# dylkot/cNMF

Hardware: AMD Instinct MI355X
Metric: NMF restarts/sec (50000x2000xK5..13) (higher is better)
Workload: dtype f32 (exact integer f16 plane x 2 f16 planes with per-row exponent, f32 accumulate)

## Files before the change

### cnmf_amd/csrc/gemm_host.hip.h

```cpp
#pragma once

struct GemmPlan { int variant; int mw; int jw; };

template <int MTW, int WM, int WN, bool NN, int TBK = BK>
static hipError_t launch_gemm_t(hipStream_t st, const float* A, int lda, const float* B, int ldb,
                                float* C, int ldc, long long cstride, int KC, int Ktot, int J,
                                int nsplit)
{
    constexpr int MW = WM * MTW * 32, JW = WN * 32;
    const int Kper = round_up((Ktot + nsplit - 1) / nsplit, BK);
    dim3 grid((J + JW - 1) / JW, KC / MW, nsplit);
    constexpr size_t lds = gemm_lds_bytes<MTW, WM, WN, NN, TBK>();
    {
        if (hipError_t e_ = dyn_lds_optin((const void*)gemm_kernel<MTW, WM, WN, NN, TBK>, (int)lds)) return e_;
    }
    gemm_kernel<MTW, WM, WN, NN, TBK><<<grid, 256, lds, st>>>(A, lda, B, ldb, C, ldc, cstride, Kper,
                                                             Ktot, J);
    return hipGetLastError();
}

static const CdKnobs k_default_knobs;
static thread_local const CdKnobs* g_knobs = &k_default_knobs;
struct KnobScope {
    const CdKnobs* prev;
    explicit KnobScope(const cnmf_ctx* ctx) : prev(g_knobs) { g_knobs = &ctx->knobs; }
    ~KnobScope() { g_knobs = prev; }
    KnobScope(const KnobScope&) = delete;
    KnobScope& operator=(const KnobScope&) = delete;
};

template <bool NN>
static hipError_t launch_gemm(hipStream_t st, int variant, const float* A, int lda, const float* B,
                              int ldb, float* C, int ldc, long long cstride, int KC, int Ktot,
                              int J, int nsplit)
{
#define GO(MTW, WM, WN) \
    return launch_gemm_t<MTW, WM, WN, NN>(st, A, lda, B, ldb, C, ldc, cstride, KC, Ktot, J, nsplit)
    if (variant == 0) variant = 2;
    if (variant == 1 && KC < 128) variant = (KC >= 64) ? 3 : 2;
    if (variant == 3 && KC < 64) variant = 2;
    switch (variant) {
        case 1:
            if (KC % 256 == 0 && KC >= 256 && g_knobs->s_mtw2) GO(2, 4, 1);
            GO(1, 4, 1);
        case 3:
            if (KC % 128 == 0) GO(2, 2, 2);
            GO(1, 2, 2);
        default:
            if (KC % 128 == 0) GO(4, 1, 4);
            if (KC % 64 == 0) GO(2, 1, 4);
            GO(1, 1, 4);
    }
#undef GO
}

static SplitInfo psum_info(int nsplit, long long stride, const double* colscale)
{
    SplitInfo sp{nullptr, reinterpret_cast<const unsigned char*>(colscale), (int)(stride >> 20), (int)(stride & ((1 << 20) - 1)), nsplit};
    return sp;
}

static hipError_t launch_sweep(hipStream_t st, int nslots, float* V, int ldv, int L, const float* P,
                               const float* gram, const SlotDesc* slots, float l1, float* gram_part,
                               double* viol_part, int chunks, int parts, int want_gram, int kmax, int tiers,
                               SplitInfo sp = SplitInfo{nullptr, nullptr, 1, 1, 1},
                               float* rmax_part = nullptr, const double* rmax_scale = nullptr, bool psum = false,
                               PlaneOut po = PlaneOut{nullptr, nullptr, 0, 0})
{
    dim3 grid(parts, nslots);
    if (po.dst) {
        if (psum || (rmax_part && rmax_scale) || (tiers & 8)) return hipErrorInvalidValue;
        const size_t pl = sweep_lds_bytes(kmax, true);
        const int kgp = sweep_kg(kmax);
        if (hipError_t e_ = dyn_lds_optin((const void*)sweep_kernel<0, false, false, true>, (int)sweep_lds_bytes(KSMALL, true))) return e_;
        if (hipError_t e_ = dyn_lds_optin((const void*)sweep_kernel<1, false, false, true>, (int)sweep_lds_bytes(KSMALL, true))) return e_;
        if (hipError_t e_ = dyn_lds_optin((const void*)sweep_kernel<2, false, false, true>, (int)sweep_lds_bytes(KSMALL, true))) return e_;
#define CNMF_SWEEP_PLN(T_) sweep_kernel<T_, false, false, true><<<grid, 256, pl, st>>>(V, ldv, L, P, sp, gram, slots, l1, gram_part, viol_part, chunks, want_gram, kgp, kmax, rmax_part, nullptr, po)
        if (tiers & 1) CNMF_SWEEP_PLN(0);
        if (tiers & 2) CNMF_SWEEP_PLN(1);
        if (tiers & 4) CNMF_SWEEP_PLN(2);
#undef CNMF_SWEEP_PLN
        return hipGetLastError();
    }
    {
        if (hipError_t e_ = dyn_lds_optin((const void*)sweep_kernel<0, false>, (int)sweep_lds_bytes(KSMALL))) return e_;
        if (hipError_t e_ = dyn_lds_optin((const void*)sweep_kernel<1, false>, (int)sweep_lds_bytes(KSMALL))) return e_;
        if (hipError_t e_ = dyn_lds_optin((const void*)sweep_kernel<2, false>, (int)sweep_lds_bytes(KSMALL))) return e_;
        if (hipError_t e_ = dyn_lds_optin((const void*)sweep_kernel<0, true>, (int)sweep_lds_bytes(KSMALL))) return e_;
        if (hipError_t e_ = dyn_lds_optin((const void*)sweep_kernel<1, true>, (int)sweep_lds_bytes(KSMALL))) return e_;
        if (hipError_t e_ = dyn_lds_optin((const void*)sweep_kernel<2, true>, (int)sweep_lds_bytes(KSMALL))) return e_;
    }
    const size_t lds = sweep_lds_bytes(kmax);
    const int kg = sweep_kg(kmax);
#define CNMF_SWEEP(T_, R_) sweep_kernel<T_, R_><<<grid, 256, lds, st>>>(V, ldv, L, P, sp, gram, slots, l1, gram_part, viol_part, chunks, want_gram, kg, kmax, rmax_part, rmax_scale)
#define CNMF_SWEEP_PSUM(T_) sweep_kernel<T_, true, true><<<grid, 256, lds, st>>>(V, ldv, L, P, sp, gram, slots, l1, gram_part, viol_part, chunks, want_gram, kg, kmax, rmax_part, rmax_scale)
    if (psum) {
        {
            if (hipError_t e_ = dyn_lds_optin((const void*)sweep_kernel<0, true, true>, (int)sweep_lds_bytes(KSMALL))) return e_;
            if (hipError_t e_ = dyn_lds_optin((const void*)sweep_kernel<1, true, true>, (int)sweep_lds_bytes(KSMALL))) return e_;
            if (hipError_t e_ = dyn_lds_optin((const void*)sweep_kernel<2, true, true>, (int)sweep_lds_bytes(KSMALL))) return e_;
        }
        if (tiers & 1) CNMF_SWEEP_PSUM(0);
        if (tiers & 2) CNMF_SWEEP_PSUM(1);
        if (tiers & 4) CNMF_SWEEP_PSUM(2);
    } else if (rmax_part && rmax_scale) {
        if (tiers & 1) CNMF_SWEEP(0, true);
        if (tiers & 2) CNMF_SWEEP(1, true);
        if (tiers & 4) CNMF_SWEEP(2, true);
    } else {
        if (tiers & 1) CNMF_SWEEP(0, false);
        if (tiers & 2) CNMF_SWEEP(1, false);
        if (tiers & 4) CNMF_SWEEP(2, false);
    }
#undef CNMF_SWEEP_PSUM
#undef CNMF_SWEEP
    if (tiers & 8) {
        if (psum) return hipErrorInvalidValue;
        const size_t blds = sweep_big_lds_bytes();
        const int bchunks = chunks;
        const dim3 gbig(parts, nslots);
        if (rmax_part && rmax_scale) {
            if (hipError_t e_ = dyn_lds_optin((const void*)sweep_big_kernel<true>, (int)blds)) return e_;
            sweep_big_kernel<true><<<gbig, 256, blds, st>>>(V, ldv, L, P, sp, gram, slots, l1, viol_part, bchunks, rmax_part, rmax_scale);
        } else {
            if (hipError_t e_ = dyn_lds_optin((const void*)sweep_big_kernel<false>, (int)blds)) return e_;
            sweep_big_kernel<false><<<gbig, 256, blds, st>>>(V, ldv, L, P, sp, gram, slots, l1, viol_part, bchunks, nullptr, nullptr);
        }
        if (want_gram)
            gram_big_kernel<<<gbig, 256, 0, st>>>(V, ldv, L, slots, gram_part, bchunks, kmax, (rmax_part && !rmax_scale) ? rmax_part : nullptr);
    }
    return hipGetLastError();
}

struct StreamK {
    bool on = false;
    int MG = 1, T = 0, nk = 0, P = 0, mw = 128;
    std::vector<unsigned char> split;
};

static StreamK plan_streamk(int KC, int N_pad, int G_pad, int n_wg_slots)
{
    StreamK sk;
    if (KC % 128 != 0 || g_knobs->no_streamk) return sk;
    sk.MG = KC / sk.mw;
    sk.T = sk.MG * (N_pad / 128);
    sk.nk = G_pad / BK;
    sk.P = n_wg_slots;
    if (sk.T <= sk.P) sk.P = n_wg_slots / 2;
    if (sk.T <= sk.P || sk.T % sk.P == 0) return sk;
    sk.on = true;
    sk.split.assign(sk.T, 0);
    const long long U = (long long)sk.T * sk.nk;
    for (int p = 1; p < sk.P; ++p) {
        const long long b = U * p / sk.P;
        if (b % sk.nk) sk.split[b / sk.nk] = 1;
    }
    return sk;
}

static hipError_t launch_streamk_passA(hipStream_t st, const StreamK& sk, const float* A, int lda,
                                       const float* B, int ldb, float* C0, float* C1, int ldc, int Jtot)
{
    constexpr size_t lds = gemm_lds_bytes<4, 1, 4, false>();
    {
        if (hipError_t e_ = dyn_lds_optin((const void*)gemm_streamk_kernel<4, 1, 4, false>, (int)lds)) return e_;
    }
    gemm_streamk_kernel<4, 1, 4, false><<<sk.P, 256, lds, st>>>(A, lda, B, ldb, C0, C1, ldc, sk.MG, sk.T,
                                                               sk.nk, Jtot);
    return hipGetLastError();
}

static hipError_t launch_reduce_splits(hipStream_t st, float* P, int nsplit, long long split_stride,
                                       long long n_floats, const double* colscale = nullptr, int ld = 1)
{
    if (nsplit <= 1 && !colscale) return hipSuccess;
    const long long nv = n_floats / 4;
    reduce_splits_kernel<<<(unsigned)((nv + 255) / 256), 256, 0, st>>>(P, nsplit, split_stride, P, nv, colscale, ld);
    return hipGetLastError();
}


static hipError_t launch_split3(hipStream_t st, const float* src, int ld, int rows, int K, unsigned char* dst, int TR,
                                const double* kscale = nullptr)
{
    if (rows % 64 == 0 && K % 64 == 0 && TR % 64 == 0) {
        dim3 grid(K / 64, rows / 64);
        split3_tiled_kernel<<<grid, 256, 0, st>>>(src, ld, K, TR, (unsigned short*)dst, kscale);
        return hipGetLastError();
    }
    const long long total = (long long)rows * (K / 16);
    split3_kernel<<<(unsigned)((total + 255) / 256), 256, 0, st>>>(src, ld, rows, K, TR, (unsigned short*)dst, kscale);
    return hipGetLastError();
}

static int gemm3_mode() { return g_knobs->gemm3; }
static int gemm3_wg_slots(const CdKnobs& k)
{
    if (k.wg_slots >= 32 && k.gemm3 >= 2) return k.wg_slots;
    return k.gemm3 >= 2 ? 256 : 512;
}
static int gemm3_jw() { return G3_JW; }

static hipError_t launch_gemm3(hipStream_t st, const unsigned char* A3, const unsigned char* B3, int Kb,
                               float* C, int ldc, long long cstride, int KC, int Jpad, int nsplit)
{
    {
        if (hipError_t e_ = dyn_lds_optin((const void*)gemm3_kernel, G3_LDS_BYTES)) return e_;
        if (hipError_t e_ = dyn_lds_optin((const void*)gemm3g_kernel, G3G_LDS_BYTES)) return e_;
    }
    const int kb_per = (Kb + nsplit - 1) / nsplit;
    dim3 grid(Jpad / gemm3_jw(), KC / G3_MW, (Kb + kb_per - 1) / kb_per);
    if (gemm3_mode() >= 2)
        gemm3g_kernel<<<grid, 512, G3G_LDS_BYTES, st>>>(A3, B3, Kb, C, ldc, cstride, kb_per);
    else
        gemm3_kernel<<<grid, 256, G3_LDS_BYTES, st>>>(A3, B3, Kb, C, ldc, cstride, kb_per);
    return hipGetLastError();
}


static hipError_t launch_split3_finalize(hipStream_t st, const float* src, int ld, int rows, int K, unsigned char* dst,
                                         int TR, const double* kscale, const FinalizeArgs& fa, int nslots, int fin_y)
{
    const int bx = K / 64, by = rows / 64;
    split3_finalize_kernel<<<bx * by + nslots * fin_y, 256, 0, st>>>(src, ld, K, TR, (unsigned short*)dst, kscale, bx, by,
                                                                  fa, fin_y);
    return hipGetLastError();
}

static hipError_t launch_split2h_finalize(hipStream_t st, const float* src, int ld, int rows, int K, unsigned char* dst,
                                          int TR, const double* kscale, const float* rmax_part, int parts,
                                          float* inv_scale, const FinalizeArgs& fa, int nslots, int fin_y,
                                          SplitFused fu = SplitFused{nullptr, nullptr});

struct StreamK3 {
    bool on = false;
    int T = 0, Kb = 0, P = 0, MG = 1;
    std::vector<unsigned char> flags;
};

static StreamK3 plan_streamk3(int KC, int N_pad, int G_pad, int n_wg_slots, int jw, int unit = 1)
{
    StreamK3 sk;
    sk.MG = KC / G3_MW;
    sk.T = sk.MG * (N_pad / jw);
    sk.Kb = G_pad / (G3_BK * unit);
    sk.P = n_wg_slots;
    if (sk.T < sk.P / 2 + sk.P / 4 || sk.P > 2 * sk.T || g_knobs->no_streamk) return sk;
    sk.on = true;
    sk.flags.assign(sk.T, 0);
    const long long U = (long long)sk.T * sk.Kb;
    const int NJ = sk.T / sk.MG;
    for (int p = 1; p < sk.P; ++p) {
        const long long b = U * p / sk.P;
        if (b % sk.Kb) {
            const int o = (int)(b / sk.Kb);
            unsigned char& f = sk.flags[(o % NJ) * sk.MG + o / NJ];
            f = f ? 3 : 1;
        }
    }
    return sk;
}
// ... 352 lines not shown
```

### cnmf_amd/csrc/kernels_sweep.hip.h

```cpp
#pragma once
#include <hip/hip_runtime.h>
#include "kernels_gemm.hip.h"
#include "kernels_gemm2h.hip.h"

namespace cnmf {

constexpr int KMAX = 128;
constexpr int KSMALL = 64;
constexpr int GRAM_LD = KMAX;
constexpr int GRAM_SZ = KMAX * KMAX;

static inline int sweep_kg(int kmax) { return kmax <= 16 ? 16 : (kmax <= 32 ? 32 : 64); }
static inline int sweep_wstride(int kmax) { return sweep_kg(kmax) + 1; }
static inline size_t sweep_lds_bytes(int kmax, bool planes = false)
{
    const int kg = sweep_kg(kmax);
    if (planes)
        return sweep_lds_bytes(kmax, false) + sizeof(float) * (size_t)(4 * kg * 64 + kg);
    return sizeof(float) * (size_t)(kg * (kg + 4) + 8 + 256 + 4 * (kg == 16 ? 32 : 64) * sweep_wstride(kmax));
}

struct SlotDesc {
    int off;
    int k;
    int active;
    int iter;
    int restart;
    int pad_;
    double viol;
    double viol_init;
    double viol_last;
};

typedef float f32x4 __attribute__((ext_vector_type(4)));

struct SplitInfo {
    const float* plane1;
    const unsigned char* split;
    int tile_rows, tile_cols, mgroups;
    const float* plane2 = nullptr;
};

struct PlaneOut {
    unsigned short* dst;
    const int* shift;
    int Kb, TR;
};

#ifndef CNMF_SWEEP_PF
#define CNMF_SWEEP_PF 0
#endif
template <int KP, bool RMX, bool PSUM = false, bool PLN = false>
__device__ __forceinline__ void sweep_body(
    float* __restrict__ V, int ldv, int L, const float* __restrict__ P, const SplitInfo& sp,
    const float* __restrict__ gram, const SlotDesc& sd, int slot, float l1_reg,
    float* __restrict__ gram_part, double* __restrict__ viol_part,
    int chunks_per_block, int want_gram, float* lds, int kg, int gld,
    float* __restrict__ rmax_part, const double* __restrict__ rmax_scale, const PlaneOut& po = PlaneOut{nullptr, nullptr, 0, 0})
{
    constexpr int GMODE = (KP <= 16) ? 0 : ((KP <= 32) ? 1 : 2);
    constexpr int GR = (GMODE == 0) ? 16 : ((GMODE == 1) ? 32 : 64);
    const int gs = kg + 4, wstride = kg + 1;
    float* Gsb = lds;
    double* vred = reinterpret_cast<double*>(lds + kg * gs);
    float* rmx = lds + kg * gs + 8;
    float* Wsb = rmx + 256;
    unsigned* Tpl = reinterpret_cast<unsigned*>(Wsb + 4 * (kg == 16 ? 32 : 64) * (kg + 1));
    int* shl = reinterpret_cast<int*>(Tpl + 4 * kg * 64);
#define GS(t_, r_) Gsb[(t_) * gs + (r_)]
    constexpr int SR = (GMODE == 0) ? 32 : 64;
#define WS(wv_, r_, c_) Wsb[((wv_) * SR + (r_)) * wstride + (c_)]
    const int k = sd.k, off = sd.off;
    const int tid = threadIdx.x, lane = tid & 63, wave = tid >> 6;
    for (int e = tid; e < KP * KP; e += 256) {
        const int r = e / KP, c = e % KP;
        GS(r, c) = (r < k && c < k) ? gram[(size_t)slot * GRAM_SZ + r * GRAM_LD + c] : 0.f;
    }
    if constexpr (PLN) { if (tid < KP) shl[tid] = po.shift[off + min(tid, k - 1)]; }
    __syncthreads();

    f32x16 gacc[GMODE == 2 ? 4 : 1];
    f32x4 gacc4 = {0.f, 0.f, 0.f, 0.f};
#pragma unroll
    for (int a = 0; a < (GMODE == 2 ? 4 : 1); ++a)
#pragma unroll
        for (int r = 0; r < 16; ++r) gacc[a][r] = 0.f;
    float viol = 0.f;
    float mx[RMX ? KP : 1];
#pragma unroll
    for (int c = 0; c < (RMX ? KP : 1); ++c) mx[c] = 0.f;

    constexpr bool PF = (CNMF_SWEEP_PF != 0) && !PSUM;
    float wn[PF ? KP : 1], pn[PF ? KP : 1];
    if constexpr (PF) {
        const int rowc0 = min((int)(blockIdx.x * chunks_per_block) * 256 + tid, L - 1);
#pragma unroll
        for (int c = 0; c < KP; ++c) {
            const size_t idx = (size_t)(off + min(c, k - 1)) * ldv + rowc0;
            wn[c] = V[idx];
            pn[c] = P[idx];
        }
    }
    for (int ch = 0; ch < chunks_per_block; ++ch) {
        const int row = (blockIdx.x * chunks_per_block + ch) * 256 + tid;
        const bool live = row < L;
        int cut0 = 0, cut1 = 0;
        int mg_edge = 1 << 30;
        if (!PSUM && sp.plane1) {
            const int rt = __builtin_amdgcn_readfirstlane(min(row, L - 1) / sp.tile_rows);
            const int g0 = off / sp.tile_cols, g1 = (off + k - 1) / sp.tile_cols;
            mg_edge = (g0 + 1) * sp.tile_cols;
            cut0 = sp.split[rt * sp.mgroups + g0];
            cut1 = sp.split[rt * sp.mgroups + g1];
        }
        float w[KP], p[KP];
        float dsc = 1.0f;
        if constexpr (RMX) { if (rmax_scale) dsc = (float)rmax_scale[min(row, L - 1)]; }
        {
            const int rowc = min(row, L - 1);
            if constexpr (PF) {
#pragma unroll
                for (int c = 0; c < KP; ++c) { w[c] = wn[c]; p[c] = pn[c]; }
                if (ch + 1 < chunks_per_block) {
                    const int rown = min(row + 256, L - 1);
#pragma unroll
                    for (int c = 0; c < KP; ++c) {
                        const size_t idx = (size_t)(off + min(c, k - 1)) * ldv + rown;
                        wn[c] = V[idx];
                        pn[c] = P[idx];
                    }
                }
            } else {
#pragma unroll
            for (int c = 0; c < KP; ++c) {
                const size_t idx = (size_t)(off + min(c, k - 1)) * ldv + rowc;
                w[c] = V[idx];
                p[c] = P[idx];
            }
            }
            if constexpr (PSUM) {
                const int nsplit = sp.mgroups;
                const size_t stride = (size_t)sp.tile_rows * (1u << 20) + (size_t)sp.tile_cols;
                constexpr int U = KP <= 16 ? 8 : (KP <= 32 ? 2 : 1);
                for (int s = 1; s < nsplit; s += U) {
                    float q[U][KP];
#pragma unroll
                    for (int u = 0; u < U; ++u) {
                        const int ss = min(s + u, nsplit - 1);
#pragma unroll
                        for (int c = 0; c < KP; ++c)
                            q[u][c] = P[ss * stride + (size_t)(off + min(c, k - 1)) * ldv + rowc];
                    }
#pragma unroll
                    for (int u = 0; u < U; ++u)
                        if (s + u < nsplit) {
#pragma unroll
                            for (int c = 0; c < KP; ++c) p[c] += q[u][c];
                        }
                }
                const double* colscale = reinterpret_cast<const double*>(sp.split);
                if (colscale) {
                    const double cs = colscale[rowc];
#pragma unroll
                    for (int c = 0; c < KP; ++c) p[c] = (float)((double)p[c] * cs);
                }
            }
            if ((cut0 | cut1) & 1) {
                float qq[KP];
#pragma unroll
                for (int c = 0; c < KP; ++c) {
                    const size_t idx = (size_t)(off + min(c, k - 1)) * ldv + rowc;
                    qq[c] = sp.plane1[idx];
                }
#pragma unroll
                for (int c = 0; c < KP; ++c) {
                    const int cut = ((off + c) < mg_edge) ? cut0 : cut1;
                    p[c] += (cut & 1) ? qq[c] : 0.f;
                }
            }
            if ((cut0 | cut1) & 2) {
                float qq[KP];
#pragma unroll
                for (int c = 0; c < KP; ++c) {
                    const size_t idx = (size_t)(off + min(c, k - 1)) * ldv + rowc;
                    qq[c] = sp.plane2[idx];
                }
#pragma unroll
                for (int c = 0; c < KP; ++c) {
                    const int cut = ((off + c) < mg_edge) ? cut0 : cut1;
                    p[c] += (cut & 2) ? qq[c] : 0.f;
                }
            }
#pragma unroll
            for (int c = 0; c < KP; ++c) {
                const bool on = live && (c < k);
                w[c] = on ? w[c] : 0.f;
                p[c] = on ? (p[c] - l1_reg) : 0.f;
            }
        }
        if (live) {
#pragma unroll
            for (int t = 0; t < KP; ++t) {
                if (t < k) {
                    float grad = -p[t];
#pragma unroll
                    for (int r = 0; r < KP; ++r) grad = fmaf(GS(t, r), w[r], grad);
                    const float pg = (w[t] == 0.f) ? fminf(0.f, grad) : grad;
                    viol += fabsf(pg);
                    const float hess = GS(t, t);
                    if (hess != 0.f) w[t] = fmaxf(w[t] - grad / hess, 0.f);
                }
            }
#pragma unroll
            for (int c = 0; c < KP; ++c)
                if (c < k) V[(size_t)(off + c) * ldv + row] = w[c];
            if constexpr (RMX) {
#pragma unroll
                for (int c = 0; c < KP; ++c) mx[c] = fmaxf(mx[c], w[c] * dsc);
            }
        }
        if (want_gram) {
            if constexpr (GMODE == 0) {
                const int li = lane & 15, q = lane >> 4;
#pragma unroll
                for (int hf = 0; hf < 2; ++hf) {
                    if ((lane >> 5) == hf) {
#pragma unroll
                        for (int c = 0; c < GR; ++c) WS(wave, lane & 31, c) = (c < KP) ? w[c < KP ? c : 0] : 0.f;
                    }
                    __builtin_amdgcn_wave_barrier();
#pragma unroll
                    for (int s = 0; s < 8; ++s) {
                        const float a = WS(wave, 4 * s + q, li);
                        gacc4 = __builtin_amdgcn_mfma_f32_16x16x4f32(a, a, gacc4, 0, 0, 0);
                    }
                    __builtin_amdgcn_wave_barrier();
                }
            } else if constexpr (GMODE == 1) {
#pragma unroll
                for (int c = 0; c < GR; ++c) WS(wave, lane, c) = (c < KP) ? w[c < KP ? c : 0] : 0.f;
                __builtin_amdgcn_wave_barrier();
                const int li = lane & 31, h = lane >> 5;
#pragma unroll 8
                for (int s = 0; s < 32; ++s) {
                    const float a = WS(wave, 2 * s + h, li);
                    gacc[0] = __builtin_amdgcn_mfma_f32_32x32x2f32(a, a, gacc[0], 0, 0, 0);
                }
            } else {
#pragma unroll
                for (int c = 0; c < GR; ++c) WS(wave, lane, c) = (c < KP) ? w[c < KP ? c : 0] : 0.f;
                __builtin_amdgcn_wave_barrier();
                const int li = lane & 31, h = lane >> 5;
#pragma unroll 4
                for (int s = 0; s < 32; ++s) {
                    const float a0 = WS(wave, 2 * s + h, li), a1 = WS(wave, 2 * s + h, 32 + li);
                    gacc[0] = __builtin_amdgcn_mfma_f32_32x32x2f32(a0, a0, gacc[0], 0, 0, 0);
                    gacc[1] = __builtin_amdgcn_mfma_f32_32x32x2f32(a0, a1, gacc[1], 0, 0, 0);
                    gacc[2] = __builtin_amdgcn_mfma_f32_32x32x2f32(a1, a0, gacc[2], 0, 0, 0);
                    gacc[3] = __builtin_amdgcn_mfma_f32_32x32x2f32(a1, a1, gacc[3], 0, 0, 0);
                }
            }
            __builtin_amdgcn_wave_barrier();
        }
        if constexpr (PLN) {
            unsigned* tw = Tpl + wave * (kg * 64);
#pragma unroll
            for (int c = 0; c < KP; ++c) {
                if (c < k) {
                    const float y = ldexpf(w[c], shl[c]);
                    unsigned short hb, mb;
                    split2h(y, hb, mb);
                    tw[c * 64 + lane] = (unsigned)hb | ((unsigned)mb << 16);
                }
            }
            __builtin_amdgcn_wave_barrier();
            const int kb0 = ((blockIdx.x * chunks_per_block + ch) * 256 + wave * 64) >> 4;
            for (int item = lane; item < 8 * k; item += 64) {
                const int c = item >> 3, b = (item >> 1) & 3, hf = item & 1;
                if (kb0 + b >= po.Kb) continue;
                const u32x4 d0 = *reinterpret_cast<const u32x4*>(tw + c * 64 + b * 16 + hf * 8);
                const u32x4 d1 = *reinterpret_cast<const u32x4*>(tw + c * 64 + b * 16 + hf * 8 + 4);
                u32x4 oh, om;
                oh.x = (d0.x & 0xffffu) | (d0.y << 16); oh.y = (d0.z & 0xffffu) | (d0.w << 16);
                oh.z = (d1.x & 0xffffu) | (d1.y << 16); oh.w = (d1.z & 0xffffu) | (d1.w << 16);
                om.x = (d0.x >> 16) | (d0.y & 0xffff0000u); om.y = (d0.z >> 16) | (d0.w & 0xffff0000u);
                om.z = (d1.x >> 16) | (d1.y & 0xffff0000u); om.w = (d1.z >> 16) | (d1.w & 0xffff0000u);
                const int r = off + c, tr = r / po.TR, rin = r % po.TR, swz = (rin >> 2) & 3;
                unsigned short* g = po.dst + (((size_t)tr * po.Kb + (kb0 + b)) * po.TR + rin) * 32;
                *reinterpret_cast<u32x4*>(g + ((0 + hf) ^ swz) * 8) = oh;
                *reinterpret_cast<u32x4*>(g + ((2 + hf) ^ swz) * 8) = om;
            }
            __builtin_amdgcn_wave_barrier();
        }
    }

    if constexpr (RMX) {
#pragma unroll
        for (int c = 0; c < KP; ++c) {
            float v = mx[c];
#pragma unroll
            for (int o = 32; o > 0; o >>= 1) v = fmaxf(v, __shfl_xor(v, o, 64));
            if (lane == 0) rmx[wave * 64 + c] = v;
        }
    }
    double dv = (double)viol;
#pragma unroll
    for (int o = 32; o > 0; o >>= 1) dv += __shfl_xor(dv, o, 64);
    if (lane == 0) vred[wave] = dv;

    __syncthreads();
    float* gred = Wsb;
    if (want_gram) {
        if constexpr (GMODE == 0) {
            const int li = lane & 15, q = lane >> 4;
#pragma unroll
            for (int r = 0; r < 4; ++r) gred[(wave * GR + 4 * q + r) * (GR + 1) + li] = gacc4[r];
        } else {
            const int li = lane & 31, h = lane >> 5;
#pragma unroll
            for (int a = 0; a < (GMODE == 2 ? 4 : 1); ++a)
#pragma unroll
                for (int r = 0; r < 16; ++r) {
                    const int rr = (a >> 1) * 32 + (r & 3) + 8 * (r >> 2) + 4 * h;
                    gred[(wave * GR + rr) * (GR + 1) + (a & 1) * 32 + li] = gacc[a][r];
                }
        }
    }
    __syncthreads();
    if (want_gram) {
        float* gp = gram_part + ((size_t)slot * gridDim.x + blockIdx.x) * (size_t)(gld * gld);
        for (int e = tid; e < k * k; e += 256) {
            const int r = e / k, c = e % k;
            gp[r * gld + c] = gred[(0 * GR + r) * (GR + 1) + c] + gred[(1 * GR + r) * (GR + 1) + c] +
                              gred[(2 * GR + r) * (GR + 1) + c] + gred[(3 * GR + r) * (GR + 1) + c];
        }
    }
    if (tid == 0)
        viol_part[(size_t)slot * gridDim.x + blockIdx.x] = vred[0] + vred[1] + vred[2] + vred[3];
    if (rmax_part && tid < k && (RMX || want_gram)) {
        float v;
        if constexpr (RMX) v = fmaxf(fmaxf(rmx[tid], rmx[64 + tid]), fmaxf(rmx[128 + tid], rmx[192 + tid]));
        else v = sqrtf(gred[(0 * GR + tid) * (GR + 1) + tid] + gred[(1 * GR + tid) * (GR + 1) + tid] +
                       gred[(2 * GR + tid) * (GR + 1) + tid] + gred[(3 * GR + tid) * (GR + 1) + tid]) * 1.0001f;
        rmax_part[(size_t)(off + tid) * gridDim.x + blockIdx.x] = v;
    }
#undef WS
#undef GS
}

template <int TIER, bool RMX = false, bool PSUM = false, bool PLN = false>
__global__ __launch_bounds__(256) __attribute__((amdgpu_waves_per_eu((TIER == 0 && !RMX && !PLN) ? 5 : (TIER == 0 && !RMX ? 4 : 1), 8))) void sweep_kernel(
    float* __restrict__ V, int ldv, int L,
    const float* __restrict__ P,
    SplitInfo sp,
    const float* __restrict__ gram,
    const SlotDesc* __restrict__ slots,
    float l1_reg,
    float* __restrict__ gram_part,
    double* __restrict__ viol_part,
    int chunks_per_block, int want_gram, int kg, int gld,
    float* __restrict__ rmax_part = nullptr,
    const double* __restrict__ rmax_scale = nullptr,
    PlaneOut po = PlaneOut{nullptr, nullptr, 0, 0})
{
    const int slot = blockIdx.y;
    const SlotDesc sd = slots[slot];
    if (!sd.active) return;
    extern __shared__ __attribute__((aligned(16))) float sweep_lds[];
#define CNMF_SW(KP_)                                                                              \
        sweep_body<KP_, RMX, PSUM, PLN>(V, ldv, L, P, sp, gram, sd, slot, l1_reg, gram_part, viol_part, \
                        chunks_per_block, want_gram, sweep_lds, kg, gld, rmax_part, rmax_scale, po);
    const int k = sd.k;
    if (TIER == 0) {
        if (k > 16) return;
        switch ((k + 3) / 4) {
            case 1: CNMF_SW(4) break;   case 2: CNMF_SW(8) break;   case 3: CNMF_SW(12) break;
            case 4: CNMF_SW(16) break;  default: break;
        }
    } else if (TIER == 1) {
        if (k <= 16 || k > 32) return;
        switch ((k + 3) / 4) {
            case 5: CNMF_SW(20) break;  case 6: CNMF_SW(24) break;
            case 7: CNMF_SW(28) break;  case 8: CNMF_SW(32) break;  default: break;
        }
    } else {
        if (k <= 32) return;
        if (k <= 48) { CNMF_SW(48) } else if (k <= 64) { CNMF_SW(64) }
    }
#undef CNMF_SW
}

constexpr int KBIG = 128;
constexpr int KBIG_GS = KBIG + 4;
static inline size_t sweep_big_lds_bytes() { return sizeof(float) * (size_t)(KBIG * KBIG_GS + 2 * 256 * 33 + 4 * KBIG + 16); }

template <bool RMX>
__global__ __launch_bounds__(256) void sweep_big_kernel(
    float* __restrict__ V, int ldv, int L, const float* __restrict__ P, SplitInfo sp, const float* __restrict__ gram,
    const SlotDesc* __restrict__ slots, float l1_reg, double* __restrict__ viol_part, int chunks_per_block,
    float* __restrict__ rmax_part, const double* __restrict__ rmax_scale)
{
    const int slot = blockIdx.y;
    const SlotDesc sd = slots[slot];
    if (!sd.active || sd.k <= KSMALL) return;
    extern __shared__ __attribute__((aligned(16))) float sweep_lds[];
    float* Gs = sweep_lds;
    float* Pl = Gs + KBIG * KBIG_GS;
    float* Wl = Pl + 256 * 33;
    float* rmx = Wl + 256 * 33;
    double* vred = reinterpret_cast<double*>(rmx + 4 * KBIG);
    const int k = sd.k, off = sd.off;
    const int tid = threadIdx.x, lane = tid & 63, wave = tid >> 6;
    for (int e = tid; e < KBIG * KBIG; e += 256) {
        const int r = e / KBIG, c = e % KBIG;
        Gs[r * KBIG_GS + c] = (r < k && c < k) ? gram[(size_t)slot * GRAM_SZ + r * GRAM_LD + c] : 0.f;
    }
    if (RMX) for (int e = tid; e < 4 * KBIG; e += 256) rmx[e] = 0.f;
    __syncthreads();
    float viol = 0.f;
    float* pl = Pl + tid * 33;
    float* wl = Wl + tid * 33;
    for (int ch = 0; ch < chunks_per_block; ++ch) {
        const int row = (blockIdx.x * chunks_per_block + ch) * 256 + tid;
        const bool live = row < L;
        const int rowc = min(row, L - 1);
        int cut0 = 0, cut1 = 0, mg_edge = 1 << 30;
        if (sp.plane1) {
            const int rt = __builtin_amdgcn_readfirstlane(rowc / sp.tile_rows);
            const int g0 = off / sp.tile_cols, g1 = (off + k - 1) / sp.tile_cols;
            mg_edge = (g0 + 1) * sp.tile_cols;
            cut0 = sp.split[rt * sp.mgroups + g0];
            cut1 = sp.split[rt * sp.mgroups + g1];
        }
        float w[KBIG];
#pragma unroll
        for (int c = 0; c < KBIG; ++c) {
            const float v = V[(size_t)(off + min(c, k - 1)) * ldv + rowc];
            w[c] = (live && c < k) ? v : 0.f;
        }
        float dsc = 1.0f;
        if (RMX && rmax_scale) dsc = (float)rmax_scale[rowc];
#pragma unroll
        for (int tb = 0; tb < KBIG / 32; ++tb) {
            if (tb * 32 < k) {
#pragma unroll
                for (int rr = 0; rr < 32; ++rr) {
                    const int c = tb * 32 + rr;
                    const size_t idx = (size_t)(off + min(c, k - 1)) * ldv + rowc;
                    float pv = P[idx];
                    const int cut = ((off + c) < mg_edge) ? cut0 : cut1;
                    if (cut & 1) pv += sp.plane1[idx];
                    if (cut & 2) pv += sp.plane2[idx];
                    pl[rr] = (live && c < k) ? pv - l1_reg : 0.f;
                    wl[rr] = w[c];
                }
                __builtin_amdgcn_wave_barrier();
                const int tend = min(32, k - tb * 32);
                for (int tt = 0; tt < tend; ++tt) {
                    const int t = tb * 32 + tt;
                    const float4* g4 = reinterpret_cast<const float4*>(Gs + t * KBIG_GS);
                    float grad = -pl[tt];
#pragma unroll
                    for (int r4 = 0; r4 < KBIG / 4; ++r4) {
                        const float4 g = g4[r4];
                        grad = fmaf(g.x, w[4 * r4 + 0], grad);
                        grad = fmaf(g.y, w[4 * r4 + 1], grad);
                        grad = fmaf(g.z, w[4 * r4 + 2], grad);
                        grad = fmaf(g.w, w[4 * r4 + 3], grad);
                    }
                    const float wt = wl[tt];
                    const float pg = (wt == 0.f) ? fminf(0.f, grad) : grad;
                    viol += live ? fabsf(pg) : 0.f;
                    const float hess = Gs[t * KBIG_GS + t];
                    float wn = wt;
                    if (hess != 0.f) wn = fmaxf(wt - grad / hess, 0.f);
#pragma unroll
                    for (int rr = 0; rr < 32; ++rr) w[tb * 32 + rr] = (rr == tt) ? wn : w[tb * 32 + rr];
                }
            }
        }
        if (live) {
#pragma unroll
            for (int c = 0; c < KBIG; ++c)
                if (c < k) V[(size_t)(off + c) * ldv + row] = w[c];
        }
        if (RMX) {
#pragma unroll
            for (int c = 0; c < KBIG; ++c) {
                if (c < k) {
                    float v = w[c] * dsc;
#pragma unroll
                    for (int o = 32; o > 0; o >>= 1) v = fmaxf(v, __shfl_xor(v, o, 64));
                    if (lane == 0) rmx[wave * KBIG + c] = fmaxf(rmx[wave * KBIG + c], v);
                }
            }
        }
    }
    double dv = (double)viol;
#pragma unroll
    for (int o = 32; o > 0; o >>= 1) dv += __shfl_xor(dv, o, 64);
    if (lane == 0) vred[wave] = dv;
    __syncthreads();
    if (tid == 0) viol_part[(size_t)slot * gridDim.x + blockIdx.x] = vred[0] + vred[1] + vred[2] + vred[3];
    if (RMX && rmax_part && tid < k)
        rmax_part[(size_t)(off + tid) * gridDim.x + blockIdx.x] =
            fmaxf(fmaxf(rmx[tid], rmx[KBIG + tid]), fmaxf(rmx[2 * KBIG + tid], rmx[3 * KBIG + tid]));
}

__global__ __launch_bounds__(256) void gram_big_kernel(const float* __restrict__ V, int ldv, int L,
                                                       const SlotDesc* __restrict__ slots, float* __restrict__ gram_part,
                                                       int chunks_per_block, int gld, float* __restrict__ rmax_part)
{
    const int slot = blockIdx.y;
    const SlotDesc sd = slots[slot];
    if (!sd.active || sd.k <= KSMALL) return;
    __shared__ float T[32][KBIG_GS];
    __shared__ float diag[KBIG];
    const int k = sd.k, off = sd.off;
    const int tid = threadIdx.x, lane = tid & 63, wave = tid >> 6;
    const int li = lane & 31, h = lane >> 5, wr = wave >> 1, wc = wave & 1;
    f32x16 acc[2][2];
#pragma unroll
    for (int i = 0; i < 2; ++i)
#pragma unroll
        for (int j = 0; j < 2; ++j)
#pragma unroll
            for (int r = 0; r < 16; ++r) acc[i][j][r] = 0.f;
    const int r_begin = blockIdx.x * chunks_per_block * 256, r_end = min(L, r_begin + chunks_per_block * 256);
    for (int r0 = r_begin; r0 < r_end; r0 += 32) {
#pragma unroll
        for (int i = 0; i < 16; ++i) {
            const int e = tid + 256 * i, c = e >> 5, rr = e & 31;
// ... 324 lines not shown
```

Baseline: 218.0.

## Use buffer loads with 32-bit offsets and exact-K specialization in sweep kernel

Non-RMX, non-PSUM sweep paths now read and write V, P and the split planes through AMD buffer resource descriptors with 32-bit offsets instead of 64-bit flat addressing. A separate A64 variant keeps flat addressing for very large ldv. Tier-0 kernels are instantiated per exact k (1..16) rather than rounded to multiples of 4, which removes padded columns, and the plane-out path uses the compile-time G3_MW tile size. The waves-per-eu hint for tier 0 with planes rises from 4 to 5. This trades many more template instantiations and larger code size for fewer address computations and less redundant work, and it relies on the buffer range check for correctness.

```diff
diff --git a/cnmf_amd/csrc/gemm_host.hip.h b/cnmf_amd/csrc/gemm_host.hip.h
--- a/cnmf_amd/csrc/gemm_host.hip.h
+++ b/cnmf_amd/csrc/gemm_host.hip.h
@@ -68,17 +68,27 @@
                                PlaneOut po = PlaneOut{nullptr, nullptr, 0, 0})
 {
     dim3 grid(parts, nslots);
+    const bool a64 = 64ll * ldv * 4 > 0x7fffffffll;
     if (po.dst) {
-        if (psum || (rmax_part && rmax_scale) || (tiers & 8)) return hipErrorInvalidValue;
+        if (psum || (rmax_part && rmax_scale) || (tiers & 8) || po.TR != G3_MW) return hipErrorInvalidValue;
         const size_t pl = sweep_lds_bytes(kmax, true);
         const int kgp = sweep_kg(kmax);
         if (hipError_t e_ = dyn_lds_optin((const void*)sweep_kernel<0, false, false, true>, (int)sweep_lds_bytes(KSMALL, true))) return e_;
         if (hipError_t e_ = dyn_lds_optin((const void*)sweep_kernel<1, false, false, true>, (int)sweep_lds_bytes(KSMALL, true))) return e_;
         if (hipError_t e_ = dyn_lds_optin((const void*)sweep_kernel<2, false, false, true>, (int)sweep_lds_bytes(KSMALL, true))) return e_;
-#define CNMF_SWEEP_PLN(T_) sweep_kernel<T_, false, false, true><<<grid, 256, pl, st>>>(V, ldv, L, P, sp, gram, slots, l1, gram_part, viol_part, chunks, want_gram, kgp, kmax, rmax_part, nullptr, po)
-        if (tiers & 1) CNMF_SWEEP_PLN(0);
-        if (tiers & 2) CNMF_SWEEP_PLN(1);
-        if (tiers & 4) CNMF_SWEEP_PLN(2);
+#define CNMF_SWEEP_PLN(T_, A_) sweep_kernel<T_, false, false, true, A_><<<grid, 256, pl, st>>>(V, ldv, L, P, sp, gram, slots, l1, gram_part, viol_part, chunks, want_gram, kgp, kmax, rmax_part, nullptr, po)
+        if (a64) {
+            if (hipError_t e_ = dyn_lds_optin((const void*)sweep_kernel<0, false, false, true, true>, (int)sweep_lds_bytes(KSMALL, true))) return e_;
+            if (hipError_t e_ = dyn_lds_optin((const void*)sweep_kernel<1, false, false, true, true>, (int)sweep_lds_bytes(KSMALL, true))) return e_;
+            if (hipError_t e_ = dyn_lds_optin((const void*)sweep_kernel<2, false, false, true, true>, (int)sweep_lds_bytes(KSMALL, true))) return e_;
+            if (tiers & 1) CNMF_SWEEP_PLN(0, true);
+            if (tiers & 2) CNMF_SWEEP_PLN(1, true);
+            if (tiers & 4) CNMF_SWEEP_PLN(2, true);
+            return hipGetLastError();
+        }
+        if (tiers & 1) CNMF_SWEEP_PLN(0, false);
+        if (tiers & 2) CNMF_SWEEP_PLN(1, false);
+        if (tiers & 4) CNMF_SWEEP_PLN(2, false);
 #undef CNMF_SWEEP_PLN
         return hipGetLastError();
     }
@@ -107,6 +117,15 @@
         if (tiers & 1) CNMF_SWEEP(0, true);
         if (tiers & 2) CNMF_SWEEP(1, true);
         if (tiers & 4) CNMF_SWEEP(2, true);
+    } else if (a64) {
+#define CNMF_SWEEP_A64(T_) sweep_kernel<T_, false, false, false, true><<<grid, 256, lds, st>>>(V, ldv, L, P, sp, gram, slots, l1, gram_part, viol_part, chunks, want_gram, kg, kmax, rmax_part, rmax_scale)
+        if (hipError_t e_ = dyn_lds_optin((const void*)sweep_kernel<0, false, false, false, true>, (int)sweep_lds_bytes(KSMALL))) return e_;
+        if (hipError_t e_ = dyn_lds_optin((const void*)sweep_kernel<1, false, false, false, true>, (int)sweep_lds_bytes(KSMALL))) return e_;
+        if (hipError_t e_ = dyn_lds_optin((const void*)sweep_kernel<2, false, false, false, true>, (int)sweep_lds_bytes(KSMALL))) return e_;
+        if (tiers & 1) CNMF_SWEEP_A64(0);
+        if (tiers & 2) CNMF_SWEEP_A64(1);
+        if (tiers & 4) CNMF_SWEEP_A64(2);
+#undef CNMF_SWEEP_A64
     } else {
         if (tiers & 1) CNMF_SWEEP(0, false);
         if (tiers & 2) CNMF_SWEEP(1, false);
diff --git a/cnmf_amd/csrc/kernels_sweep.hip.h b/cnmf_amd/csrc/kernels_sweep.hip.h
--- a/cnmf_amd/csrc/kernels_sweep.hip.h
+++ b/cnmf_amd/csrc/kernels_sweep.hip.h
@@ -47,10 +47,7 @@
     int Kb, TR;
 };
 
-#ifndef CNMF_SWEEP_PF
-#define CNMF_SWEEP_PF 0
-#endif
-template <int KP, bool RMX, bool PSUM = false, bool PLN = false>
+template <int KP, bool RMX, bool PSUM = false, bool PLN = false, bool EX = false, bool B32 = false>
 __device__ __forceinline__ void sweep_body(
     float* __restrict__ V, int ldv, int L, const float* __restrict__ P, const SplitInfo& sp,
     const float* __restrict__ gram, const SlotDesc& sd, int slot, float l1_reg,
@@ -60,7 +57,7 @@
 {
     constexpr int GMODE = (KP <= 16) ? 0 : ((KP <= 32) ? 1 : 2);
     constexpr int GR = (GMODE == 0) ? 16 : ((GMODE == 1) ? 32 : 64);
-    const int gs = kg + 4, wstride = kg + 1;
+    const int gs = EX ? 20 : kg + 4, wstride = kg + 1;
     float* Gsb = lds;
     double* vred = reinterpret_cast<double*>(lds + kg * gs);
     float* rmx = lds + kg * gs + 8;
@@ -70,8 +67,13 @@
 #define GS(t_, r_) Gsb[(t_) * gs + (r_)]
     constexpr int SR = (GMODE == 0) ? 32 : 64;
 #define WS(wv_, r_, c_) Wsb[((wv_) * SR + (r_)) * wstride + (c_)]
-    const int k = sd.k, off = sd.off;
+    static_assert(!(B32 && PSUM) && !(EX && KP > 16), "sweep_body: EX is tier 0, B32 has no PSUM form");
+    const int k = EX ? KP : sd.k, off = sd.off;
     const int tid = threadIdx.x, lane = tid & 63, wave = tid >> 6;
+    const unsigned slot_bytes = B32 ? (unsigned)k * (unsigned)ldv * 4u : 0u;
+    const int col_bytes = ldv * 4;
+#define CNMF_RSRC(ptr_) __builtin_amdgcn_make_buffer_rsrc((void*)((ptr_) + (size_t)off * ldv), 0, (int)slot_bytes, 0x00020000)
+#define CNMF_BLD(rs_, voff_, c_) __builtin_bit_cast(float, __builtin_amdgcn_raw_buffer_load_b32(rs_, voff_, min(c_, k - 1) * col_bytes, 0))
     for (int e = tid; e < KP * KP; e += 256) {
         const int r = e / KP, c = e % KP;
         GS(r, c) = (r < k && c < k) ? gram[(size_t)slot * GRAM_SZ + r * GRAM_LD + c] : 0.f;
@@ -90,17 +92,6 @@
 #pragma unroll
     for (int c = 0; c < (RMX ? KP : 1); ++c) mx[c] = 0.f;
 
-    constexpr bool PF = (CNMF_SWEEP_PF != 0) && !PSUM;
-    float wn[PF ? KP : 1], pn[PF ? KP : 1];
-    if constexpr (PF) {
-        const int rowc0 = min((int)(blockIdx.x * chunks_per_block) * 256 + tid, L - 1);
-#pragma unroll
-        for (int c = 0; c < KP; ++c) {
-            const size_t idx = (size_t)(off + min(c, k - 1)) * ldv + rowc0;
-            wn[c] = V[idx];
-            pn[c] = P[idx];
-        }
-    }
     for (int ch = 0; ch < chunks_per_block; ++ch) {
         const int row = (blockIdx.x * chunks_per_block + ch) * 256 + tid;
         const bool live = row < L;
@@ -118,25 +109,22 @@
         if constexpr (RMX) { if (rmax_scale) dsc = (float)rmax_scale[min(row, L - 1)]; }
         {
             const int rowc = min(row, L - 1);
-            if constexpr (PF) {
-#pragma unroll
-                for (int c = 0; c < KP; ++c) { w[c] = wn[c]; p[c] = pn[c]; }
-                if (ch + 1 < chunks_per_block) {
-                    const int rown = min(row + 256, L - 1);
-#pragma unroll
-                    for (int c = 0; c < KP; ++c) {
-                        const size_t idx = (size_t)(off + min(c, k - 1)) * ldv + rown;
-                        wn[c] = V[idx];
-                        pn[c] = P[idx];
-                    }
+            const int voff = rowc * 4;
+            if constexpr (B32) {
+                const auto rV = CNMF_RSRC(V);
+                const auto rP = CNMF_RSRC(P);
+#pragma unroll
+                for (int c = 0; c < KP; ++c) {
+                    w[c] = CNMF_BLD(rV, voff, c);
+                    p[c] = CNMF_BLD(rP, voff, c);
                 }
             } else {
 #pragma unroll
-            for (int c = 0; c < KP; ++c) {
-                const size_t idx = (size_t)(off + min(c, k - 1)) * ldv + rowc;
-                w[c] = V[idx];
-                p[c] = P[idx];
-            }
+                for (int c = 0; c < KP; ++c) {
+                    const size_t idx = (size_t)(off + min(c, k - 1)) * ldv + rowc;
+                    w[c] = V[idx];
+                    p[c] = P[idx];
+                }
             }
             if constexpr (PSUM) {
                 const int nsplit = sp.mgroups;
@@ -167,10 +155,16 @@
             }
             if ((cut0 | cut1) & 1) {
                 float qq[KP];
-#pragma unroll
-                for (int c = 0; c < KP; ++c) {
-                    const size_t idx = (size_t)(off + min(c, k - 1)) * ldv + rowc;
-                    qq[c] = sp.plane1[idx];
+                if constexpr (B32) {
+                    const auto r1 = CNMF_RSRC(sp.plane1);
+#pragma unroll
+                    for (int c = 0; c < KP; ++c) qq[c] = CNMF_BLD(r1, voff, c);
+                } else {
+#pragma unroll
+                    for (int c = 0; c < KP; ++c) {
+                        const size_t idx = (size_t)(off + min(c, k - 1)) * ldv + rowc;
+                        qq[c] = sp.plane1[idx];
+                    }
                 }
 #pragma unroll
                 for (int c = 0; c < KP; ++c) {
@@ -180,10 +174,16 @@
             }
             if ((cut0 | cut1) & 2) {
                 float qq[KP];
-#pragma unroll
-                for (int c = 0; c < KP; ++c) {
-                    const size_t idx = (size_t)(off + min(c, k - 1)) * ldv + rowc;
-                    qq[c] = sp.plane2[idx];
+                if constexpr (B32) {
+                    const auto r2 = CNMF_RSRC(sp.plane2);
+#pragma unroll
+                    for (int c = 0; c < KP; ++c) qq[c] = CNMF_BLD(r2, voff, c);
+                } else {
+#pragma unroll
+                    for (int c = 0; c < KP; ++c) {
+                        const size_t idx = (size_t)(off + min(c, k - 1)) * ldv + rowc;
+                        qq[c] = sp.plane2[idx];
+                    }
                 }
 #pragma unroll
                 for (int c = 0; c < KP; ++c) {
@@ -211,22 +211,31 @@
                     if (hess != 0.f) w[t] = fmaxf(w[t] - grad / hess, 0.f);
                 }
             }
-#pragma unroll
-            for (int c = 0; c < KP; ++c)
-                if (c < k) V[(size_t)(off + c) * ldv + row] = w[c];
+            if constexpr (B32) {
+                const auto rV = CNMF_RSRC(V);
+#pragma unroll
+                for (int c = 0; c < KP; ++c)
+                    if (c < k) __builtin_amdgcn_raw_buffer_store_b32(__builtin_bit_cast(unsigned, w[c]), rV, row * 4, c * col_bytes, 0);
+            } else {
+#pragma unroll
+                for (int c = 0; c < KP; ++c)
+                    if (c < k) V[(size_t)(off + c) * ldv + row] = w[c];
+            }
             if constexpr (RMX) {
 #pragma unroll
                 for (int c = 0; c < KP; ++c) mx[c] = fmaxf(mx[c], w[c] * dsc);
             }
         }
+        int ln = lane;
+        if constexpr (EX) asm volatile("" : "+v"(ln));
         if (want_gram) {
             if constexpr (GMODE == 0) {
-                const int li = lane & 15, q = lane >> 4;
+                const int li = ln & 15, q = ln >> 4;
 #pragma unroll
                 for (int hf = 0; hf < 2; ++hf) {
-                    if ((lane >> 5) == hf) {
-#pragma unroll
-                        for (int c = 0; c < GR; ++c) WS(wave, lane & 31, c) = (c < KP) ? w[c < KP ? c : 0] : 0.f;
+                    if ((ln >> 5) == hf) {
+#pragma unroll
+                        for (int c = 0; c < GR; ++c) WS(wave, ln & 31, c) = (c < KP) ? w[c < KP ? c : 0] : 0.f;
                     }
                     __builtin_amdgcn_wave_barrier();
 #pragma unroll
@@ -270,12 +279,12 @@
                     const float y = ldexpf(w[c], shl[c]);
                     unsigned short hb, mb;
                     split2h(y, hb, mb);
-                    tw[c * 64 + lane] = (unsigned)hb | ((unsigned)mb << 16);
+                    tw[c * 64 + ln] = (unsigned)hb | ((unsigned)mb << 16);
                 }
             }
             __builtin_amdgcn_wave_barrier();
             const int kb0 = ((blockIdx.x * chunks_per_block + ch) * 256 + wave * 64) >> 4;
-            for (int item = lane; item < 8 * k; item += 64) {
+            for (int item = ln; item < 8 * k; item += 64) {
                 const int c = item >> 3, b = (item >> 1) & 3, hf = item & 1;
                 if (kb0 + b >= po.Kb) continue;
                 const u32x4 d0 = *reinterpret_cast<const u32x4*>(tw + c * 64 + b * 16 + hf * 8);
@@ -285,8 +294,8 @@
                 oh.z = (d1.x & 0xffffu) | (d1.y << 16); oh.w = (d1.z & 0xffffu) | (d1.w << 16);
                 om.x = (d0.x >> 16) | (d0.y & 0xffff0000u); om.y = (d0.z >> 16) | (d0.w & 0xffff0000u);
                 om.z = (d1.x >> 16) | (d1.y & 0xffff0000u); om.w = (d1.z >> 16) | (d1.w & 0xffff0000u);
-                const int r = off + c, tr = r / po.TR, rin = r % po.TR, swz = (rin >> 2) & 3;
-                unsigned short* g = po.dst + (((size_t)tr * po.Kb + (kb0 + b)) * po.TR + rin) * 32;
+                const int r = off + c, tr = r / G3_MW, rin = r % G3_MW, swz = (rin >> 2) & 3;
+                unsigned short* g = po.dst + (((size_t)tr * po.Kb + (kb0 + b)) * G3_MW + rin) * 32;
                 *reinterpret_cast<u32x4*>(g + ((0 + hf) ^ swz) * 8) = oh;
                 *reinterpret_cast<u32x4*>(g + ((2 + hf) ^ swz) * 8) = om;
             }
@@ -344,12 +353,14 @@
                        gred[(2 * GR + tid) * (GR + 1) + tid] + gred[(3 * GR + tid) * (GR + 1) + tid]) * 1.0001f;
         rmax_part[(size_t)(off + tid) * gridDim.x + blockIdx.x] = v;
     }
+#undef CNMF_BLD
+#undef CNMF_RSRC
 #undef WS
 #undef GS
 }
 
-template <int TIER, bool RMX = false, bool PSUM = false, bool PLN = false>
-__global__ __launch_bounds__(256) __attribute__((amdgpu_waves_per_eu((TIER == 0 && !RMX && !PLN) ? 5 : (TIER == 0 && !RMX ? 4 : 1), 8))) void sweep_kernel(
+template <int TIER, bool RMX = false, bool PSUM = false, bool PLN = false, bool A64 = false>
+__global__ __launch_bounds__(256) __attribute__((amdgpu_waves_per_eu((TIER == 0 && !RMX) ? 5 : 1, 8))) void sweep_kernel(
     float* __restrict__ V, int ldv, int L,
     const float* __restrict__ P,
     SplitInfo sp,
@@ -367,17 +378,29 @@
     const SlotDesc sd = slots[slot];
     if (!sd.active) return;
     extern __shared__ __attribute__((aligned(16))) float sweep_lds[];
+    static_assert(!A64 || (!RMX && !PSUM), "A64 is the flat-address form of the W half-step kernels");
+    constexpr bool B32 = !RMX && !PSUM && !A64, EX = B32 && TIER == 0;
 #define CNMF_SW(KP_)                                                                              \
-        sweep_body<KP_, RMX, PSUM, PLN>(V, ldv, L, P, sp, gram, sd, slot, l1_reg, gram_part, viol_part, \
+        sweep_body<KP_, RMX, PSUM, PLN, EX, B32>(V, ldv, L, P, sp, gram, sd, slot, l1_reg, gram_part, viol_part, \
                         chunks_per_block, want_gram, sweep_lds, kg, gld, rmax_part, rmax_scale, po);
     const int k = sd.k;
-    if (TIER == 0) {
+    if constexpr (TIER == 0) {
         if (k > 16) return;
-        switch ((k + 3) / 4) {
-            case 1: CNMF_SW(4) break;   case 2: CNMF_SW(8) break;   case 3: CNMF_SW(12) break;
-            case 4: CNMF_SW(16) break;  default: break;
-        }
-    } else if (TIER == 1) {
+        if constexpr (EX) {
+            switch (k) {
+                case 1: CNMF_SW(1) break;    case 2: CNMF_SW(2) break;    case 3: CNMF_SW(3) break;    case 4: CNMF_SW(4) break;
+                case 5: CNMF_SW(5) break;    case 6: CNMF_SW(6) break;    case 7: CNMF_SW(7) break;    case 8: CNMF_SW(8) break;
+                case 9: CNMF_SW(9) break;    case 10: CNMF_SW(10) break;  case 11: CNMF_SW(11) break;  case 12: CNMF_SW(12) break;
+                case 13: CNMF_SW(13) break;  case 14: CNMF_SW(14) break;  case 15: CNMF_SW(15) break;  case 16: CNMF_SW(16) break;
+                default: break;
+            }
+        } else {
+            switch ((k + 3) / 4) {
+                case 1: CNMF_SW(4) break;   case 2: CNMF_SW(8) break;   case 3: CNMF_SW(12) break;
+                case 4: CNMF_SW(16) break;  default: break;
+            }
+        }
+    } else if constexpr (TIER == 1) {
         if (k <= 16 || k > 32) return;
         switch ((k + 3) / 4) {
             case 5: CNMF_SW(20) break;  case 6: CNMF_SW(24) break;
```

Result: faster. 221.0 (median of 6 runs) (+1.3%).
